# TianyiFranklinWang/MIRROR

Hardware: AMD Instinct MI355X
Metric: SSL samples/sec (slide+RNA pairs) (higher is better)
Workload: dtype bf16; 1 GPU; BASELINE c2: B=16/GPU x [4096 patch tokens x 1024-d] + [2048 genes], D=512, RNA depth 6 / 8 heads, train mode, local-batch InfoNCE; precision_policy=bf16, per_gpu_batch=16, global_batch=16, parallelism=dp1, grad_bucket_dtype=f32, step_launch=hip_graph

## Files before the change

### include/mirror_hip.h

```cpp
#ifndef MIRROR_HIP_H
#define MIRROR_HIP_H
#include <stdint.h>

#ifdef __cplusplus
extern "C" {
#endif

#define MH_OK 0
#define MH_EINVAL (-1)
#define MH_EUNSUP (-2)
#define MH_EHIP (-3)

#define MH_F32 0
#define MH_BF16 1

#define MH_ACT_NONE 0
#define MH_ACT_RELU 1
#define MH_ACT_GELU 2

typedef void* mh_stream;

const char* mh_last_error(void);
int mh_version(void);
int mh_exp_build(void);
// ... 197 lines not shown
    float* stats;
    void* qkv;
    float* attn;
    void* o;
    float* x1;
    void* u;
    void* f;
    const float* dy;
    float* dx;
    float *dw_qkv, *dw_proj, *dw_fc1, *dw_fc2, *db_qkv, *db_proj, *db_fc1, *db_fc2, *dg1, *dbe1, *dg2, *dbe2;
    void* scratch;
} mh_rna_block;
int mh_rna_block_fwd(const mh_rna_block* blk, mh_stream s);
int mh_rna_block_bwd(const mh_rna_block* blk, mh_stream s);
int64_t mh_rna_block_workspace_bytes(int B, int D, int Hh);

int mh_headattn_fwd(const void* qkv, void* out, float* attn, int B, int H, int hd, int dt, mh_stream s);
int mh_headattn_bwd(const void* qkv, const float* attn, const void* dout, void* dqkv, int B, int H, int hd,
                    int dt, mh_stream s);

int mh_add(const void* a, const void* b, void* y, int64_t n, int dt_a, int dt_b, int dt_y, mh_stream s);
int mh_cast(const void* x, void* y, int64_t n, int dt_x, int dt_y, mh_stream s);
int mh_gelu_fwd(const void* x, void* y, int64_t n, int dt_x, int dt_y, mh_stream s);
int mh_gelu_bwd(const void* x, const void* dy, void* dx, int64_t n, int dt_x, int dt_dy, int dt_dx, mh_stream s);
int mh_relu_bwd(const void* y, const void* dy, void* dx, int64_t n_per_batch, int batches, int64_t y_bs, int64_t dy_bs,
                int64_t dx_bs, int dt_y, int dt_dy, int dt_dx, mh_stream s);
int mh_noise_draws(float* out, int64_t n_uniform, int64_t n_normal, uint64_t seed, uint64_t offset, const uint64_t* dev_base, mh_stream s);
int mh_dropout(const void* x, void* y, int64_t n, float p, uint64_t seed, uint64_t offset, const uint64_t* dev_base,
               int dt_x, int dt_y, mh_stream s);
int mh_dropout_add(const float* a, const void* x, float* y, int64_t n, float p, uint64_t seed, uint64_t offset,
// ... 186 lines not shown
```

### mirror_amd/_lib.py

```python
from __future__ import annotations

import ctypes as C
import os

_HERE = os.path.dirname(os.path.abspath(__file__))
LIB_PATH = os.environ.get("MIRROR_HIP_LIB") or os.path.join(_HERE, "lib", "libmirror_hip.so")

MH_F32, MH_BF16 = 0, 1
ACT_NONE, ACT_RELU, ACT_GELU = 0, 1, 2


class GemmEpi(C.Structure):
    _fields_ = [
        ("kind", C.c_int32), ("resid", C.c_void_p),
        ("p", C.c_float), ("seed", C.c_uint64), ("offset", C.c_uint64), ("dev_base", C.c_void_p),
        ("mask", C.c_void_p), ("token", C.c_void_p), ("pos", C.c_void_p),
        ("rows_per_batch", C.c_int32), ("first", C.c_int32),
        ("tgt", C.c_void_p), ("tgt_bs", C.c_int64), ("sq", C.c_void_p),
    ]


class SkinnyWgradItem(C.Structure):
    _fields_ = [("dy", C.c_void_p), ("lddy", C.c_int64), ("x", C.c_void_p), ("ldx", C.c_int64), ("dw", C.c_void_p), ("lddw", C.c_int64),
                ("db", C.c_void_p), ("M", C.c_int32), ("N", C.c_int32), ("K", C.c_int32), ("dt_dy", C.c_int32), ("dt_x", C.c_int32)]
# ... 159 lines not shown
    "mh_kl_fwd": [P, P, P, L, F],
    "mh_kl_bwd": [P, P, P, P, P, L, F],
    "mh_symkl_fwd": [P, P, P, I, I, F],
    "mh_symkl_bwd": [P, P, P, P, P, I, I, F],
    "mh_rownorm_": [P, P, I, I, F],
    "mh_clamp_": [P, L, F, F],
    "mh_adam": [P, P, P, P, P, L, F, F, F, F, F, F, F, P, L, F, F, P, L, I, L, L],
    "mh_adam_ema": [P, P, P, P, P, L, F, F, F, F, F, F, F, P, L, F, F, P, L, I, L, L, P, P],
    "mh_ema_update_many": [P, P, I, F, P, P],
    "mh_optim_step": [P, P, P, P, P, L, P, P, P, I, F, P, L, F, F, P, L, I, L, L, P, P],
    "mh_optim_groups": [P, P, P, P, P, L, P, P, P, P, I, F, P, L, F, F, P, L, I, L, L, P, P],
    "mh_gather_many": [P, P, I],
    "mh_grad_clip": [P, L, F, F, P, P],
    "mh_rna_block_fwd": [C.POINTER(RnaBlockDesc)],
    "mh_rna_block_bwd": [C.POINTER(RnaBlockDesc)],
    "mh_loss_terms_fwd": [C.POINTER(LossTermsDesc)],
    "mh_loss_terms_bwd": [C.POINTER(LossTermsDesc)],
    "mh_surv_loss_fwd": [P, L, P, I, P, I, I, I, I, F, F, F, F, F, P, P],
    "mh_surv_loss_bwd": [P, L, P, I, P, I, I, I, I, F, F, F, F, P, I, F, P],
    "mh_surv_risk": [P, L, I, I, P],
    "mh_cindex_counts": [P, P, P, L, F, P],
    "mh_cls_ce_fwd": [P, L, P, I, I, I, F, L, P, P, I],
    "mh_cls_ce_bwd": [P, L, P, I, I, I, F, L, P, I, P],
    "mh_cls_confusion": [P, L, I, P, I, I, I, P, P],
    "mh_auroc_counts": [P, L, P, I, I, P],
    "mh_infonce_paired_fwd": [P, P, P, P, I, I, I, F, I],
    "mh_infonce_paired_bwd": [P, P, P, P, P, P, P, I, I, I, I, I],
    "mh_infonce_rows_fwd": [P, P, P, L, I, I, I, F, F, P, P, P, P],
    "mh_infonce_rows_bwd": [P, L, P, P, P, I, F, F, I, I, P, P],
    "mh_infonce_fold": [P, P, P, P, I, P, P, I, I],
# ... 107 lines not shown
```

### mirror_amd/csrc/rna_block.hip

```cpp
#include "common.h"

typedef __bf16 rb_bf16x8 __attribute__((ext_vector_type(8)));
typedef float rb_f4 __attribute__((ext_vector_type(4)));
typedef unsigned rb_u4 __attribute__((ext_vector_type(4)));
typedef unsigned rb_u2 __attribute__((ext_vector_type(2)));

namespace {

constexpr int PADK = 8;

struct Drop {
    float p;
    unsigned long long seed, offset;
};

__device__ __forceinline__ rb_f4 drop4(const Drop& d, long i) {
    if (d.p <= 0.f) return rb_f4{1.f, 1.f, 1.f, 1.f};
    const float scale = 1.f / (1.f - d.p);
    const uint32_t thr = (uint32_t)fminf(d.p * 4294967296.f, 4294967295.f);
    const uint64_t blk = (d.offset + (uint64_t)i) >> 2;
    uint32_t ctr[4] = {(uint32_t)blk, (uint32_t)(blk >> 32), 0u, 0u};
    philox4x32_10(ctr, (uint32_t)d.seed, (uint32_t)(d.seed >> 32));
    return rb_f4{ctr[0] >= thr ? scale : 0.f, ctr[1] >= thr ? scale : 0.f, ctr[2] >= thr ? scale : 0.f, ctr[3] >= thr ? scale : 0.f};
}
// ... 201 lines not shown
    Drop drop;
    int B, M;
    const bf16_t* wt;
    int Kin, epi;
    void* dx;
    const bf16_t* u;
    Drop drop2;
    int xsrc;
    const bf16_t* x_in;
    const float *xl, *stats_l, *gamma_l, *beta_l;
    float *dw, *db;
    const unsigned long long* dev_base;
    int n_dgrad, n_wgrad;
};

__device__ __forceinline__ rb_f4 gval4(const BwdArgs& g, const float* c12, int m, int n) {
    const long idx = (long)m * g.M + n;
    if (g.src == 0) return unpack4(*reinterpret_cast<const rb_u2*>(g.g_in + idx));
    rb_f4 v = *reinterpret_cast<const rb_f4*>(g.r + idx);
    if (g.src == 2) {
        const float mean = g.stats[m], rstd = g.stats[g.B + m];
        const rb_f4 xh = (*reinterpret_cast<const rb_f4*>(g.xs + idx) - mean) * rstd;
        const rb_f4 a = *reinterpret_cast<const rb_f4*>(g.dh + idx) * *reinterpret_cast<const rb_f4*>(g.gamma + n);
        v += rstd * (a - c12[m] - xh * c12[32 + m]);
    }
    return v;
}

template <int MT, int QPL>
__global__ __launch_bounds__(256) void rna_bwd_kernel(BwdArgs g) {
    extern __shared__ __attribute__((aligned(16))) char smem[];
    __shared__ float c12[64];
    const int lane = threadIdx.x & 63, wave = threadIdx.x >> 6;
    const int M = g.M;
    if (g.dev_base) {
        const unsigned long long base = *g.dev_base & ~3ull;
        g.drop.offset += base;
        g.drop2.offset += base;
    }
    const int role = (int)blockIdx.x < g.n_dgrad ? 0 : ((int)blockIdx.x < g.n_dgrad + g.n_wgrad ? 1 : 2);
// ... 15 lines not shown
                        dbt += dv[i];
                    }
            }
            g.dgamma[n] += dg;
            g.dbeta[n] += dbt;
        }
        return;
    }
    const int k0 = blockIdx.x * 16;
    const bf16_t* wp = nullptr;
    WPre pre;
    if (role == 0) {
        wp = wfrag_ptr(g.wt, M, k0, g.Kin);
        wfrag_batch(pre, wp, M / 32, wave);
    }
    if (g.src == 2) {
        for (int i0 = 0; i0 < MT * 4; i0 += 4) {
            rb_f4 xv[4][QPL], dv[4][QPL], gm[QPL];
#pragma unroll
            for (int j = 0; j < QPL; j++) {
                const int n = min(4 * (lane + 64 * j), M - 4);
                gm[j] = *reinterpret_cast<const rb_f4*>(g.gamma + n);
#pragma unroll
                for (int i = 0; i < 4; i++) {
                    const long idx = (long)min(wave + 4 * (i0 + i), g.B - 1) * M + n;
                    xv[i][j] = *reinterpret_cast<const rb_f4*>(g.xs + idx);
                    dv[i][j] = *reinterpret_cast<const rb_f4*>(g.dh + idx);
                }
            }
#pragma unroll
            for (int i = 0; i < 4; i++) {
// ... 7 lines not shown
                        s1 += a[0] + a[1] + a[2] + a[3];
                        s2 += a[0] * xh[0] + a[1] * xh[1] + a[2] * xh[2] + a[3] * xh[3];
                    }
                s1 = wave_sum(s1) / (float)M;
                s2 = wave_sum(s2) / (float)M;
                if (lane == 0 && wave + 4 * (i0 + i) < g.B) { c12[m] = s1; c12[32 + m] = s2; }
            }
        }
        __syncthreads();
    }
    if (role == 0) {
        bf16_t* sG = reinterpret_cast<bf16_t*>(smem);
        const int pitch = M + PADK;
        float* red = reinterpret_cast<float*>(smem + (size_t)MT * 16 * pitch * 2);
        const int nchunk = (M + 256 * QPL - 1) / (256 * QPL);
        for (int i0 = 0; i0 < MT * 4; i0 += 4)
            for (int c = 0; c < nchunk; c++) {
                rb_f4 v[4][QPL];
#pragma unroll
                for (int i = 0; i < 4; i++)
#pragma unroll
                    for (int j = 0; j < QPL; j++) {
                        const int m = min(wave + 4 * (i0 + i), g.B - 1), n = min(256 * QPL * c + 4 * (lane + 64 * j), M - 4);
                        v[i][j] = gval4(g, c12, m, n);
                    }
#pragma unroll
                for (int i = 0; i < 4; i++)
#pragma unroll
                    for (int j = 0; j < QPL; j++) {
                        const int m = wave + 4 * (i0 + i), n = 256 * QPL * c + 4 * (lane + 64 * j);
                        if (n >= M) continue;
                        rb_f4 o = {0.f, 0.f, 0.f, 0.f};
                        if (m < g.B) o = v[i][j] * drop4(g.drop, (long)m * M + n);
                        *reinterpret_cast<rb_u2*>(sG + m * pitch + n) = pack4(o);
                        if (g.src == 2 && g.r_out && m < g.B && (n >> 4) == (int)blockIdx.x) *reinterpret_cast<rb_f4*>(g.r_out + (long)m * M + n) = v[i][j];
                    }
            }
        __syncthreads();
        skinny_core<MT>(sG, M, wp, pre, red);
        __syncthreads();
        for (int i = threadIdx.x; i < MT * 64; i += 256) {
            const int t = i >> 6, rr = (i >> 2) & 15, c4 = 4 * (i & 3);
            const int m = 16 * t + rr, k = k0 + c4;
            if (m >= g.B || k >= g.Kin) continue;
            rb_f4 v = red_quad<MT>(red, t, rr, c4);
            const long idx = (long)m * g.Kin + k;
            if (g.epi == 1) {
                const rb_f4 uu = unpack4(*reinterpret_cast<const rb_u2*>(g.u + idx));
                v *= drop4(g.drop2, idx) * rb_f4{gelu_grad_f(uu[0]), gelu_grad_f(uu[1]), gelu_grad_f(uu[2]), gelu_grad_f(uu[3])};
            }
// ... 70 lines not shown
    }
    if (kt0 + 8 * tk >= g.Kin) return;
#pragma unroll
    for (int i = 0; i < 8; i++) {
        const int n = n0 + 8 * tn + i;
        if (n >= M) continue;
        float* dst = g.dw + (long)n * g.Kin + kt0 + 8 * tk;
        rb_f4 o0 = {acc[i][0], acc[i][1], acc[i][2], acc[i][3]}, o1 = {acc[i][4], acc[i][5], acc[i][6], acc[i][7]};
        o0 += *reinterpret_cast<const rb_f4*>(dst);
        o1 += *reinterpret_cast<const rb_f4*>(dst + 4);
        *reinterpret_cast<rb_f4*>(dst) = o0;
        *reinterpret_cast<rb_f4*>(dst + 4) = o1;
    }
}

int launch_bwd(BwdArgs a, hipStream_t s) {
    const int MT = a.B <= 16 ? 1 : 2;
    a.n_dgrad = a.dx ? mh_cdiv(a.Kin, 16) : 0;
    a.n_wgrad = a.dw ? mh_cdiv(a.M, 64) * mh_cdiv(a.Kin, 256) : 0;
    const int n_wgrad = a.n_wgrad + (a.src == 2 ? 1 : 0);
    const size_t lds_d = (size_t)MT * 16 * (a.M + PADK) * 2 + (size_t)4 * MT * 16 * 17 * 4, lds_w = 32 * 64 * 4 + 32 * 256 * 4;
    const size_t lds = lds_d > lds_w ? lds_d : lds_w;
    dim3 grid(a.n_dgrad + n_wgrad);
    if (grid.x == 0) return 0;
    static const bool attr = [] {
#define RNA_A(MT_, Q_) (void)hipFuncSetAttribute(reinterpret_cast<const void*>(&rna_bwd_kernel<MT_, Q_>), hipFuncAttributeMaxDynamicSharedMemorySize, 158 * 1024)
        RNA_A(1, 2); RNA_A(1, 4); RNA_A(1, 8); RNA_A(2, 2); RNA_A(2, 4); RNA_A(2, 8);
#undef RNA_A
        return true;
    }();
    (void)attr;
    if (lds > 158 * 1024) { mh_set_error("rna block: operand image of %zu bytes exceeds the 160 KiB of LDS", lds); return MH_EINVAL; }
#define RNA_B(MT_, Q_) hipLaunchKernelGGL((rna_bwd_kernel<MT_, Q_>), grid, dim3(256), lds, s, a)
    const int q = a.M <= 512 ? 2 : (a.M <= 1024 ? 4 : 8);
    if (MT == 1) { if (q == 2) RNA_B(1, 2); else if (q == 4) RNA_B(1, 4); else RNA_B(1, 8); }
    else { if (q == 2) RNA_B(2, 2); else if (q == 4) RNA_B(2, 4); else RNA_B(2, 8); }
#undef RNA_B
// ... 51 lines not shown
            dbt += d;
            dx[idx] = (r ? r[idx] : 0.f) + rstd * (d * gmn - c12[m] - xh * c12[32 + m]);
        }
    }
    part[0][wave][lane] = dg;
    part[1][wave][lane] = dbt;
    __syncthreads();
    if (wave == 0 && n < D) {
        dgamma[n] += part[0][0][lane] + part[0][1][lane] + part[0][2][lane] + part[0][3][lane];
        dbeta[n] += part[1][0][lane] + part[1][1][lane] + part[1][2][lane] + part[1][3][lane];
    }
}

inline long q4(long n) { return (n + 3) / 4 * 4; }

}

extern "C" int64_t mh_rna_block_workspace_bytes(int B, int D, int Hh) {
    auto al = [](long n) { return (n + 255) / 256 * 256; };
    return al(2L * B * Hh) + 3 * al(4L * B * D) + al(2L * B * D) + al(6L * B * D);
}

static int rna_check(const mh_rna_block* b, const char* who) {
    MH_REQUIRE(b, "%s: null descriptor", who);
    MH_REQUIRE(b->B >= 1 && b->B <= 32, "%s: B=%d (needs 1..32 rows)", who, b->B);
    MH_REQUIRE(b->D % 32 == 0 && b->Hh % 32 == 0 && b->D > 0 && b->Hh > 0, "%s: D=%d, Hh=%d must be multiples of 32", who, b->D, b->Hh);
    MH_REQUIRE(b->H >= 1 && b->H <= 64 && b->D % b->H == 0 && b->D <= 4096, "%s: H=%d does not divide D=%d", who, b->H, b->D);
    MH_REQUIRE(b->Hh <= 4096 && b->D <= 2048, "%s: D=%d, Hh=%d exceed the batched prologues (D <= 2048, Hh <= 4096)", who, b->D, b->Hh);
    MH_REQUIRE(b->p_drop >= 0.f && b->p_drop < 1.f && (b->offset & 3) == 0, "%s: bad dropout arguments", who);
    return MH_OK;
}

extern "C" int mh_rna_block_fwd(const mh_rna_block* b, mh_stream s) {
    if (int rc = rna_check(b, "mh_rna_block_fwd")) return rc;
    hipStream_t st = (hipStream_t)s;
    const int B = b->B, D = b->D, Hh = b->Hh;
    const unsigned long long base = b->offset;
    const Drop none{0.f, 0ull, 0ull};
    Drop d1{b->p_drop, b->seed, base}, d2{b->p_drop, b->seed, base + q4((long)B * D)}, d3{b->p_drop, b->seed, base + q4((long)B * D) + q4((long)B * Hh)};
    FwdArgs a{};
    a.B = B;
    a.dev_base = (const unsigned long long*)b->dev_base;
    a.a = b->x; a.a_f32 = 1; a.ln = 1; a.gamma = b->g1; a.beta = b->be1; a.eps = b->eps; a.stats = b->stats;
    a.w = (const bf16_t*)b->w_qkv; a.bias = b->b_qkv; a.out = b->qkv; a.out_f32 = 0; a.preact = nullptr; a.res = nullptr; a.act = MH_ACT_NONE;
    a.drop = none; a.N = 3 * D; a.K = D;
    if (int rc = launch_fwd(a, st)) return rc;
    if (int rc = mh_headattn_fwd(b->qkv, b->o, b->attn, B, b->H, D / b->H, MH_BF16, s)) return rc;
    a.a = b->o; a.a_f32 = 0; a.ln = 0; a.stats = nullptr; a.w = (const bf16_t*)b->w_proj; a.bias = b->b_proj; a.out = b->x1; a.out_f32 = 1;
    a.res = b->x; a.drop = d1; a.N = D; a.K = D;
    if (int rc = launch_fwd(a, st)) return rc;
    a.a = b->x1; a.a_f32 = 1; a.ln = 1; a.gamma = b->g2; a.beta = b->be2; a.stats = b->stats + 2 * B;
    a.w = (const bf16_t*)b->w_fc1; a.bias = b->b_fc1; a.out = b->f; a.out_f32 = 0; a.preact = (bf16_t*)b->u; a.res = nullptr; a.act = MH_ACT_GELU;
    a.drop = d2; a.N = Hh; a.K = D;
    if (int rc = launch_fwd(a, st)) return rc;
    a.a = b->f; a.a_f32 = 0; a.ln = 0; a.stats = nullptr; a.w = (const bf16_t*)b->w_fc2; a.bias = b->b_fc2; a.out = b->y; a.out_f32 = 1;
    a.preact = nullptr; a.res = b->x1; a.act = MH_ACT_NONE; a.drop = d3; a.N = D; a.K = Hh;
    if (int rc = launch_fwd(a, st)) return rc;
    MH_LAUNCH_CHECK("mh_rna_block_fwd");
    return MH_OK;
}

extern "C" int mh_rna_block_bwd(const mh_rna_block* b, mh_stream s) {
    if (int rc = rna_check(b, "mh_rna_block_bwd")) return rc;
    MH_REQUIRE(b->scratch && b->dy && b->dx, "mh_rna_block_bwd: dy, dx and scratch are required");
    hipStream_t st = (hipStream_t)s;
    const int B = b->B, D = b->D, Hh = b->Hh;
    auto al = [](long n) { return (n + 255) / 256 * 256; };
    char* ws = (char*)b->scratch;
    bf16_t* dg = (bf16_t*)ws; ws += al(2L * B * Hh);
    float* dh2 = (float*)ws; ws += al(4L * B * D);
    float* dx1 = (float*)ws; ws += al(4L * B * D);
    bf16_t* dO = (bf16_t*)ws; ws += al(2L * B * D);
    bf16_t* dqkv = (bf16_t*)ws; ws += al(6L * B * D);
    float* dh1 = (float*)ws;
    const Drop none{0.f, 0ull, 0ull};
    Drop d1{b->p_drop, b->seed, b->offset}, d2{b->p_drop, b->seed, b->offset + q4((long)B * D)},
        d3{b->p_drop, b->seed, b->offset + q4((long)B * D) + q4((long)B * Hh)};
    BwdArgs a{};
    a.dev_base = (const unsigned long long*)b->dev_base;
    a.B = B;
    a.src = 1; a.r = b->dy; a.drop = d3; a.M = D; a.wt = (const bf16_t*)b->wt_fc2; a.Kin = Hh; a.epi = 1; a.dx = dg; a.u = (const bf16_t*)b->u; a.drop2 = d2;
    a.xsrc = 0; a.x_in = (const bf16_t*)b->f; a.dw = b->dw_fc2; a.db = b->db_fc2;
    if (int rc = launch_bwd(a, st)) return rc;
    a = BwdArgs{};
    a.dev_base = (const unsigned long long*)b->dev_base;
    a.B = B; a.src = 0; a.g_in = dg; a.drop = none; a.M = Hh; a.wt = (const bf16_t*)b->wt_fc1; a.Kin = D; a.epi = 0; a.dx = dh2; a.drop2 = none;
    a.xsrc = 1; a.xl = b->x1; a.stats_l = b->stats + 2 * B; a.gamma_l = b->g2; a.beta_l = b->be2; a.dw = b->dw_fc1; a.db = b->db_fc1;
    if (int rc = launch_bwd(a, st)) return rc;
    a = BwdArgs{};
    a.dev_base = (const unsigned long long*)b->dev_base;
    a.B = B; a.src = 2; a.r = b->dy; a.dh = dh2; a.xs = b->x1; a.stats = b->stats + 2 * B; a.gamma = b->g2; a.r_out = dx1; a.dgamma = b->dg2; a.dbeta = b->dbe2;
    a.drop = d1; a.M = D; a.wt = (const bf16_t*)b->wt_proj; a.Kin = D; a.epi = 2; a.dx = dO; a.drop2 = none;
    a.xsrc = 0; a.x_in = (const bf16_t*)b->o; a.dw = b->dw_proj; a.db = b->db_proj;
    if (int rc = launch_bwd(a, st)) return rc;
    if (int rc = mh_headattn_bwd(b->qkv, b->attn, dO, dqkv, B, b->H, D / b->H, MH_BF16, s)) return rc;
    a = BwdArgs{};
    a.dev_base = (const unsigned long long*)b->dev_base;
    a.B = B; a.src = 0; a.g_in = dqkv; a.drop = none; a.M = 3 * D; a.wt = (const bf16_t*)b->wt_qkv; a.Kin = D; a.epi = 0; a.dx = dh1; a.drop2 = none;
    a.xsrc = 1; a.xl = b->x; a.stats_l = b->stats; a.gamma_l = b->g1; a.beta_l = b->be1; a.dw = b->dw_qkv; a.db = b->db_qkv;
    if (int rc = launch_bwd(a, st)) return rc;
#define RNA_L(Q_) hipLaunchKernelGGL((rna_ln_bwd_res_kernel<Q_>), dim3(mh_cdiv(D, 64)), dim3(256), 0, st, (const float*)dx1, (const float*)dh1, b->x, (const float*)b->stats, b->g1, b->dx, b->dg1, b->dbe1, B, D)
    if (D <= 512) RNA_L(2); else if (D <= 1024) RNA_L(4); else RNA_L(8);
#undef RNA_L
    MH_LAUNCH_CHECK("mh_rna_block_bwd");
    return MH_OK;
}
```

### mirror_amd/functional.py

```python
from __future__ import annotations

from dataclasses import dataclass
from typing import List, Optional, Tuple

import os

import torch
from torch.autograd import Function

from . import kernels as K
from ._lib import ACT_NONE, ACT_RELU, MH_BF16, MH_F32

f32, bf16 = torch.float32, torch.bfloat16


@dataclass(frozen=True)
class Precision:
    name: str
    mma: int
    act: torch.dtype
    pinv_mma: int
    fp8_fwd: bool = False


# ... 2080 lines not shown
        ctx.H = H
        return out

    @staticmethod
    def backward(ctx, dout):
        qkv, attn = ctx.saved_tensors
        dout = dout.contiguous()
        if dout.dtype != qkv.dtype:
            dout = K.cast(dout, qkv.dtype)
        return K.headattn_bwd(qkv, attn, dout, ctx.H), None


_RNA_FUSED = True


class RnaBlockFn(Function):

    NAMES = ("g1", "be1", "w_qkv", "b_qkv", "w_proj", "b_proj", "g2", "be2", "w_fc1", "b_fc1", "w_fc2", "b_fc2")

    @staticmethod
    def forward(ctx, x, g1, be1, wqkv, bqkv, wproj, bproj, g2, be2, w1, b1, w2, b2, H, eps, p, prec):
        masters = dict(zip(RnaBlockFn.NAMES, (g1, be1, wqkv, bqkv, wproj, bproj, g2, be2, w1, b1, w2, b2)))
        params = {}
        for k, v in masters.items():
            if v is None:
                params[k] = None
            elif k.startswith("w_"):
                params[k] = shadow(v, prec).contiguous()
            else:
                params[k] = v.detach().reshape(-1)
        B, D = x.shape
        Hh = w1.shape[0]
        st = _dropout_state
        ctx.drop = (float(p), st["seed"], st["offset"], st["base"]) if p > 0.0 else (0.0, 0, 0, None)
        if p > 0.0:
            q4 = lambda n: (n + 3) // 4 * 4
            o0 = st["offset"]
            st["offset"] += 2 * q4(B * D) + q4(B * Hh)
            _tap((B, D), p, st["seed"], o0, False)
            _tap((B, Hh), p, st["seed"], o0 + q4(B * D), False)
            _tap((B, D), p, st["seed"], o0 + q4(B * D) + q4(B * Hh), False)
        y, saved = K.rna_block_fwd(x, params, H, eps, *ctx.drop)
        ctx.masters, ctx.saved, ctx.cfg = masters, saved, (H, eps, prec)
        ctx.save_for_backward(x)
        return y

    @staticmethod
    def backward(ctx, dy):
        (x,) = ctx.saved_tensors
        H, eps, prec = ctx.cfg
        masters = ctx.masters
        params, params_t, grads, rets = {}, {}, {}, {}
        for k, v in masters.items():
            if v is None:
                params[k] = None
                continue
            if k.startswith("w_"):
                params[k] = shadow(v, prec).contiguous()
                params_t["wt_" + k[2:]] = shadow_t(v, prec)
                gk = "dw_" + k[2:]
            else:
                params[k] = v.detach().reshape(-1)
                gk = {"g1": "dg1", "be1": "dbe1", "g2": "dg2", "be2": "dbe2"}.get(k, "d" + k)
            buf, sunk = _gbuf(v, tuple(v.shape))
            grads[gk] = buf
            rets[k] = (v, buf, sunk)
        dx = K.rna_block_bwd(x, dy.contiguous().float(), params, params_t, grads, ctx.saved, H, eps, *ctx.drop)
        out = [dx]
        for k in RnaBlockFn.NAMES:
            if k in rets:
                v, buf, sunk = rets[k]
                out.append(_gret(v, buf, sunk))
            else:
                out.append(None)
        return tuple(out) + (None, None, None, None)


def rna_block(x, blk, prec: Precision, training: bool):
    a, m = blk.attn, blk.mlp
    p = float(a.proj_drop) if training else 0.0
    if not (_RNA_FUSED and prec.act == bf16 and x.dtype == f32 and K.rna_block_ok(x, x.shape[-1], m.fc1.weight.shape[0], a.num_heads)
            and float(m.drop) == float(a.proj_drop) and blk.norm1.eps == blk.norm2.eps):
        return None
    return RnaBlockFn.apply(x.contiguous(), blk.norm1.weight, blk.norm1.bias, a.qkv.weight, a.qkv.bias, a.proj.weight, a.proj.bias,
                            blk.norm2.weight, blk.norm2.bias, m.fc1.weight, m.fc1.bias, m.fc2.weight, m.fc2.bias,
                            a.num_heads, float(blk.norm1.eps), p, prec)


class ExpFn(Function):

    @staticmethod
    def forward(ctx, x):
        y = K.exp_fwd(x.detach().contiguous())
        ctx.save_for_backward(y)
        ctx.x = x
        return y

    @staticmethod
    def backward(ctx, dy):
        (y,) = ctx.saved_tensors
        dx, sunk = _gbuf_n(ctx.x, tuple(y.shape))
# ... 407 lines not shown
```

### mirror_amd/kernels.py

```python
from __future__ import annotations

import ctypes as C
import os
from typing import Optional


import torch

from . import _lib
from ._lib import ACT_GELU, ACT_NONE, ACT_RELU, MH_BF16, MH_F32, GemmDesc, MirrorHipError

_DT = {torch.float32: MH_F32, torch.bfloat16: MH_BF16}


def dt(t: torch.Tensor) -> int:
    try:
        return _DT[t.dtype]
    except KeyError:
        raise MirrorHipError(f"unsupported dtype {t.dtype} (f32 / bf16 only)") from None


_raw_stream = getattr(torch._C, "_cuda_getCurrentRawStream", None)


# ... 1273 lines not shown

def rna_block_bwd(x, dy, params: dict, params_t: dict, grads: dict, saved: dict, H: int, eps: float, p: float, seed: int, offset: int,
                  dev_base) -> torch.Tensor:
    import ctypes
    B, D = x.shape
    Hh = params["w_fc1"].shape[0]
    if dy.dtype != torch.float32 or not dy.is_contiguous() or dy.shape != x.shape:
        raise MirrorHipError("rna_block_bwd: dy must be a contiguous f32 [B, D] tensor")
    dx = torch.empty_like(x)
    scratch = torch.empty((rna_block_workspace_bytes(B, D, Hh),), device=x.device, dtype=torch.uint8)
    d = _rna_desc(B, D, Hh, H, eps, p, seed, offset, dev_base, x=x, dy=dy, dx=dx, scratch=scratch, **params, **params_t, **grads, **saved)
    _lib.call("mh_rna_block_bwd", ctypes.byref(d), stream=_stream())
    return dx


def add(a: torch.Tensor, b: torch.Tensor, out_dtype=None, out: Optional[torch.Tensor] = None) -> torch.Tensor:
    _chk(a, b, out)
    _contig(a, "add a"), _contig(b, "add b")
    if a.shape != b.shape:
        raise MirrorHipError(f"add: shapes differ {tuple(a.shape)} vs {tuple(b.shape)}")
    y = out if out is not None else torch.empty_like(a, dtype=out_dtype or a.dtype)
    _lib.call("mh_add", _p(a), _p(b), _p(y), a.numel(), dt(a), dt(b), dt(y), stream=_stream())
    return y


def lm_merge(a: torch.Tensor, b: Optional[torch.Tensor], out2: torch.Tensor, zero_cols: int) -> None:
    _chk(a, b, out2)
    rows, cols = a.numel() // a.shape[-1], a.shape[-1]
    if not (a.dtype == torch.float32 and a.is_contiguous() and (b is None or (b.dtype == torch.float32 and b.is_contiguous() and b.numel() == a.numel()))
            and out2.dim() == 2 and out2.dtype == torch.bfloat16 and out2.stride(1) == 1 and tuple(out2.shape) == (rows, cols + zero_cols)):
# ... 851 lines not shown
```

### mirror_amd/models/mirror.py

```python
from __future__ import annotations

import logging
import math
import os
from typing import Dict, Optional, Tuple

import numpy as np
import torch
from torch import nn

from .. import functional as Fn
from ..functional import FP32, BF16, POLICIES, Precision
from .._lib import ACT_NONE, MirrorHipError

_logger = logging.getLogger(__name__)
f32 = torch.float32

_DEFAULT_PRECISION: Optional[str] = None

_LM_MASKED = True


def set_precision(name: Optional[str]) -> None:
    global _DEFAULT_PRECISION
# ... 92 lines not shown
        if not gene_embed or gene_embed == "none":
            self.gene_embed = None
        else:
            self.gene_embed = nn.Parameter(torch.randn(1, embed_dim) * 0.02)
            _trunc_normal_(self.gene_embed, std=0.02)
        self.pos_drop_rate = pos_drop_rate
        self.blocks = nn.Sequential(*[
            Block(embed_dim, num_heads, mlp_ratio, qkv_bias, proj_drop_rate, norm_eps) for _ in range(depth)])
        self.norm = nn.LayerNorm(embed_dim, eps=norm_eps)
        self.precision: Optional[str] = None

    def forward(self, x):
        prec = resolve_precision(self.precision)
        x = self.embedding(x, prec, extra_bias=self.gene_embed, out_dtype=f32)
        x = Fn.dropout(x, self.pos_drop_rate, self.training)
        for blk in self.blocks:
            x = blk(x, prec)
        return Fn.layer_norm(x, self.norm.weight, self.norm.bias, self.norm.eps, out_dtype=f32)


class NystromAttention(nn.Module):

    def __init__(self, dim, dim_head=64, heads=8, num_landmarks=256, pinv_iterations=6, residual=True,
                 residual_conv_kernel=33, eps=1e-8, dropout=0.0):
        super().__init__()
        assert residual, "the reference always enables the residual conv (models/mirror.py:306)"
        inner = heads * dim_head
        self.heads, self.num_landmarks, self.pinv_iterations = heads, num_landmarks, pinv_iterations
        self.eps, self.drop = eps, dropout
        self.to_qkv = nn.Linear(dim, inner * 3, bias=False)
        self.to_out = nn.Sequential(nn.Linear(inner, dim), nn.Dropout(dropout))
        ks = residual_conv_kernel
# ... 503 lines not shown
```

Baseline: 2229 samples/s.

## Fuse RNA transformer blocks into one stack call with cross-block LN-backward join

Replaces the per-block autograd function for the RNA transformer with a single stacked function that runs all blocks forward in one library call. In backward, each block's closing layernorm-backward kernel is dropped: its residual join is folded into the next-lower block's first backward kernel, which reads the upper block's dx1 and dh1 scratch. For small rows it adds a one-pass path that computes the LN reduction and the join together. This cuts per-block kernel launches and one round trip of activation gradients through memory. The cost is a separate scratch buffer per block and more complex descriptor bookkeeping, though under hip_graph launch overhead is already low.

```diff
diff --git a/include/mirror_hip.h b/include/mirror_hip.h
--- a/include/mirror_hip.h
+++ b/include/mirror_hip.h
@@ -235,6 +235,8 @@
 int mh_rna_block_fwd(const mh_rna_block* blk, mh_stream s);
 int mh_rna_block_bwd(const mh_rna_block* blk, mh_stream s);
 int64_t mh_rna_block_workspace_bytes(int B, int D, int Hh);
+int mh_rna_stack_fwd(const mh_rna_block* blks, int L, mh_stream s);
+int mh_rna_stack_bwd(const mh_rna_block* blks, int L, mh_stream s);
 
 int mh_headattn_fwd(const void* qkv, void* out, float* attn, int B, int H, int hd, int dt, mh_stream s);
 int mh_headattn_bwd(const void* qkv, const float* attn, const void* dout, void* dqkv, int B, int H, int hd,
diff --git a/mirror_amd/_lib.py b/mirror_amd/_lib.py
--- a/mirror_amd/_lib.py
+++ b/mirror_amd/_lib.py
@@ -197,6 +197,8 @@
     "mh_grad_clip": [P, L, F, F, P, P],
     "mh_rna_block_fwd": [C.POINTER(RnaBlockDesc)],
     "mh_rna_block_bwd": [C.POINTER(RnaBlockDesc)],
+    "mh_rna_stack_fwd": [C.POINTER(RnaBlockDesc), I],
+    "mh_rna_stack_bwd": [C.POINTER(RnaBlockDesc), I],
     "mh_loss_terms_fwd": [C.POINTER(LossTermsDesc)],
     "mh_loss_terms_bwd": [C.POINTER(LossTermsDesc)],
     "mh_surv_loss_fwd": [P, L, P, I, P, I, I, I, I, F, F, F, F, F, P, P],
diff --git a/mirror_amd/csrc/rna_block.hip b/mirror_amd/csrc/rna_block.hip
--- a/mirror_amd/csrc/rna_block.hip
+++ b/mirror_amd/csrc/rna_block.hip
@@ -239,16 +239,19 @@
     int n_dgrad, n_wgrad;
 };
 
+__device__ __forceinline__ rb_f4 ln_join(rb_f4 r, rb_f4 x, rb_f4 dh, rb_f4 gamma, float mean, float rstd, float c1, float c2) {
+    const rb_f4 xh = (x - mean) * rstd;
+    const rb_f4 a = dh * gamma;
+    return r + rstd * (a - c1 - xh * c2);
+}
+
 __device__ __forceinline__ rb_f4 gval4(const BwdArgs& g, const float* c12, int m, int n) {
     const long idx = (long)m * g.M + n;
     if (g.src == 0) return unpack4(*reinterpret_cast<const rb_u2*>(g.g_in + idx));
     rb_f4 v = *reinterpret_cast<const rb_f4*>(g.r + idx);
-    if (g.src == 2) {
-        const float mean = g.stats[m], rstd = g.stats[g.B + m];
-        const rb_f4 xh = (*reinterpret_cast<const rb_f4*>(g.xs + idx) - mean) * rstd;
-        const rb_f4 a = *reinterpret_cast<const rb_f4*>(g.dh + idx) * *reinterpret_cast<const rb_f4*>(g.gamma + n);
-        v += rstd * (a - c12[m] - xh * c12[32 + m]);
-    }
+    if (g.src == 2)
+        v = ln_join(v, *reinterpret_cast<const rb_f4*>(g.xs + idx), *reinterpret_cast<const rb_f4*>(g.dh + idx),
+                    *reinterpret_cast<const rb_f4*>(g.gamma + n), g.stats[m], g.stats[g.B + m], c12[m], c12[32 + m]);
     return v;
 }
 
@@ -294,7 +297,8 @@
         wp = wfrag_ptr(g.wt, M, k0, g.Kin);
         wfrag_batch(pre, wp, M / 32, wave);
     }
-    if (g.src == 2) {
+    constexpr bool ONE_PASS = QPL <= 2;
+    if (g.src == 2 && !(ONE_PASS && role == 0)) {
         for (int i0 = 0; i0 < MT * 4; i0 += 4) {
             rb_f4 xv[4][QPL], dv[4][QPL], gm[QPL];
 #pragma unroll
@@ -332,6 +336,48 @@
         const int pitch = M + PADK;
         float* red = reinterpret_cast<float*>(smem + (size_t)MT * 16 * pitch * 2);
         const int nchunk = (M + 256 * QPL - 1) / (256 * QPL);
+        if (ONE_PASS && g.src == 2) {
+            for (int i0 = 0; i0 < MT * 4; i0 += 4) {
+                rb_f4 xv[4][QPL], dv[4][QPL], rv[4][QPL], gm[QPL];
+#pragma unroll
+                for (int j = 0; j < QPL; j++) {
+                    const int n = min(4 * (lane + 64 * j), M - 4);
+                    gm[j] = *reinterpret_cast<const rb_f4*>(g.gamma + n);
+#pragma unroll
+                    for (int i = 0; i < 4; i++) {
+                        const long idx = (long)min(wave + 4 * (i0 + i), g.B - 1) * M + n;
+                        xv[i][j] = *reinterpret_cast<const rb_f4*>(g.xs + idx);
+                        dv[i][j] = *reinterpret_cast<const rb_f4*>(g.dh + idx);
+                        rv[i][j] = *reinterpret_cast<const rb_f4*>(g.r + idx);
+                    }
+                }
+#pragma unroll
+                for (int i = 0; i < 4; i++) {
+                    const int m = wave + 4 * (i0 + i), mc = min(m, g.B - 1);
+                    const float mean = g.stats[mc], rstd = g.stats[g.B + mc];
+                    float s1 = 0.f, s2 = 0.f;
+#pragma unroll
+                    for (int j = 0; j < QPL; j++)
+                        if (4 * (lane + 64 * j) < M) {
+                            const rb_f4 xh = (xv[i][j] - mean) * rstd, a = dv[i][j] * gm[j];
+                            s1 += a[0] + a[1] + a[2] + a[3];
+                            s2 += a[0] * xh[0] + a[1] * xh[1] + a[2] * xh[2] + a[3] * xh[3];
+                        }
+                    s1 = wave_sum(s1) / (float)M;
+                    s2 = wave_sum(s2) / (float)M;
+#pragma unroll
+                    for (int j = 0; j < QPL; j++) {
+                        const int n = 4 * (lane + 64 * j);
+                        if (n >= M) continue;
+                        const rb_f4 v = ln_join(rv[i][j], xv[i][j], dv[i][j], gm[j], mean, rstd, s1, s2);
+                        rb_f4 o = {0.f, 0.f, 0.f, 0.f};
+                        if (m < g.B) o = v * drop4(g.drop, (long)m * M + n);
+                        *reinterpret_cast<rb_u2*>(sG + m * pitch + n) = pack4(o);
+                        if (g.r_out && m < g.B && (n >> 4) % g.n_dgrad == (int)blockIdx.x) *reinterpret_cast<rb_f4*>(g.r_out + (long)m * M + n) = v;
+                    }
+                }
+            }
+        } else
         for (int i0 = 0; i0 < MT * 4; i0 += 4)
             for (int c = 0; c < nchunk; c++) {
                 rb_f4 v[4][QPL];
@@ -351,7 +397,7 @@
                         rb_f4 o = {0.f, 0.f, 0.f, 0.f};
                         if (m < g.B) o = v[i][j] * drop4(g.drop, (long)m * M + n);
                         *reinterpret_cast<rb_u2*>(sG + m * pitch + n) = pack4(o);
-                        if (g.src == 2 && g.r_out && m < g.B && (n >> 4) == (int)blockIdx.x) *reinterpret_cast<rb_f4*>(g.r_out + (long)m * M + n) = v[i][j];
+                        if (g.src == 2 && g.r_out && m < g.B && (n >> 4) % g.n_dgrad == (int)blockIdx.x) *reinterpret_cast<rb_f4*>(g.r_out + (long)m * M + n) = v[i][j];
                     }
             }
         __syncthreads();
@@ -452,13 +498,18 @@
     }
 }
 
+size_t bwd_lds(int B, int M) {
+    const int MT = B <= 16 ? 1 : 2;
+    const size_t lds_d = (size_t)MT * 16 * (M + PADK) * 2 + (size_t)4 * MT * 16 * 17 * 4, lds_w = 32 * 64 * 4 + 32 * 256 * 4;
+    return lds_d > lds_w ? lds_d : lds_w;
+}
+
 int launch_bwd(BwdArgs a, hipStream_t s) {
     const int MT = a.B <= 16 ? 1 : 2;
     a.n_dgrad = a.dx ? mh_cdiv(a.Kin, 16) : 0;
     a.n_wgrad = a.dw ? mh_cdiv(a.M, 64) * mh_cdiv(a.Kin, 256) : 0;
     const int n_wgrad = a.n_wgrad + (a.src == 2 ? 1 : 0);
-    const size_t lds_d = (size_t)MT * 16 * (a.M + PADK) * 2 + (size_t)4 * MT * 16 * 17 * 4, lds_w = 32 * 64 * 4 + 32 * 256 * 4;
-    const size_t lds = lds_d > lds_w ? lds_d : lds_w;
+    const size_t lds = bwd_lds(a.B, a.M);
     dim3 grid(a.n_dgrad + n_wgrad);
     if (grid.x == 0) return 0;
     static const bool attr = [] {
@@ -540,12 +591,27 @@
 
 inline long q4(long n) { return (n + 3) / 4 * 4; }
 
-}
-
-extern "C" int64_t mh_rna_block_workspace_bytes(int B, int D, int Hh) {
-    auto al = [](long n) { return (n + 255) / 256 * 256; };
-    return al(2L * B * Hh) + 3 * al(4L * B * D) + al(2L * B * D) + al(6L * B * D);
-}
+struct Ws {
+    bf16_t *dg, *dO, *dqkv;
+    float *dh2, *dx1, *dh1, *dyj;
+    long bytes;
+    Ws(void* scratch, int B, int D, int Hh) {
+        auto al = [](long n) { return (n + 255) / 256 * 256; };
+        char* p = (char*)scratch;
+        dg = (bf16_t*)p; p += al(2L * B * Hh);
+        dh2 = (float*)p; p += al(4L * B * D);
+        dx1 = (float*)p; p += al(4L * B * D);
+        dO = (bf16_t*)p; p += al(2L * B * D);
+        dqkv = (bf16_t*)p; p += al(6L * B * D);
+        dh1 = (float*)p; p += al(4L * B * D);
+        dyj = (float*)p; p += al(4L * B * D);
+        bytes = p - (char*)scratch;
+    }
+};
+
+}
+
+extern "C" int64_t mh_rna_block_workspace_bytes(int B, int D, int Hh) { return Ws(nullptr, B, D, Hh).bytes; }
 
 static int rna_check(const mh_rna_block* b, const char* who) {
     MH_REQUIRE(b, "%s: null descriptor", who);
@@ -557,8 +623,8 @@
     return MH_OK;
 }
 
-extern "C" int mh_rna_block_fwd(const mh_rna_block* b, mh_stream s) {
-    if (int rc = rna_check(b, "mh_rna_block_fwd")) return rc;
+static int rna_fwd_one(const mh_rna_block* b, mh_stream s, const char* who) {
+    if (int rc = rna_check(b, who)) return rc;
     hipStream_t st = (hipStream_t)s;
     const int B = b->B, D = b->D, Hh = b->Hh;
     const unsigned long long base = b->offset;
@@ -581,31 +647,47 @@
     if (int rc = launch_fwd(a, st)) return rc;
     a.a = b->f; a.a_f32 = 0; a.ln = 0; a.stats = nullptr; a.w = (const bf16_t*)b->w_fc2; a.bias = b->b_fc2; a.out = b->y; a.out_f32 = 1;
     a.preact = nullptr; a.res = b->x1; a.act = MH_ACT_NONE; a.drop = d3; a.N = D; a.K = Hh;
-    if (int rc = launch_fwd(a, st)) return rc;
+    return launch_fwd(a, st);
+}
+
+extern "C" int mh_rna_block_fwd(const mh_rna_block* b, mh_stream s) {
+    if (int rc = rna_fwd_one(b, s, "mh_rna_block_fwd")) return rc;
     MH_LAUNCH_CHECK("mh_rna_block_fwd");
     return MH_OK;
 }
 
-extern "C" int mh_rna_block_bwd(const mh_rna_block* b, mh_stream s) {
-    if (int rc = rna_check(b, "mh_rna_block_bwd")) return rc;
-    MH_REQUIRE(b->scratch && b->dy && b->dx, "mh_rna_block_bwd: dy, dx and scratch are required");
+extern "C" int mh_rna_stack_fwd(const mh_rna_block* blks, int L, mh_stream s) {
+    MH_REQUIRE(blks && L >= 1, "mh_rna_stack_fwd: needs at least one block");
+    for (int l = 0; l < L; l++) {
+        MH_REQUIRE(l == 0 || blks[l].x == blks[l - 1].y, "mh_rna_stack_fwd: block %d does not read block %d's output", l, l - 1);
+        if (int rc = rna_fwd_one(blks + l, s, "mh_rna_stack_fwd")) return rc;
+    }
+    MH_LAUNCH_CHECK("mh_rna_stack_fwd");
+    return MH_OK;
+}
+
+static int rna_bwd_one(const mh_rna_block* b, const mh_rna_block* above, bool close, mh_stream s, const char* who) {
+    if (int rc = rna_check(b, who)) return rc;
+    MH_REQUIRE(b->scratch && (above || b->dy) && (!close || b->dx), "%s: dy, dx and scratch are required", who);
+    MH_REQUIRE(!above || (above->B == b->B && above->D == b->D && above->scratch), "%s: stacked blocks differ in B or D", who);
     hipStream_t st = (hipStream_t)s;
     const int B = b->B, D = b->D, Hh = b->Hh;
-    auto al = [](long n) { return (n + 255) / 256 * 256; };
-    char* ws = (char*)b->scratch;
-    bf16_t* dg = (bf16_t*)ws; ws += al(2L * B * Hh);
-    float* dh2 = (float*)ws; ws += al(4L * B * D);
-    float* dx1 = (float*)ws; ws += al(4L * B * D);
-    bf16_t* dO = (bf16_t*)ws; ws += al(2L * B * D);
-    bf16_t* dqkv = (bf16_t*)ws; ws += al(6L * B * D);
-    float* dh1 = (float*)ws;
+    const Ws w(b->scratch, B, D, Hh);
+    bf16_t *dg = w.dg, *dO = w.dO, *dqkv = w.dqkv;
+    float *dh2 = w.dh2, *dx1 = w.dx1, *dh1 = w.dh1;
+    const float* dy = above ? w.dyj : b->dy;
     const Drop none{0.f, 0ull, 0ull};
     Drop d1{b->p_drop, b->seed, b->offset}, d2{b->p_drop, b->seed, b->offset + q4((long)B * D)},
         d3{b->p_drop, b->seed, b->offset + q4((long)B * D) + q4((long)B * Hh)};
     BwdArgs a{};
     a.dev_base = (const unsigned long long*)b->dev_base;
     a.B = B;
-    a.src = 1; a.r = b->dy; a.drop = d3; a.M = D; a.wt = (const bf16_t*)b->wt_fc2; a.Kin = Hh; a.epi = 1; a.dx = dg; a.u = (const bf16_t*)b->u; a.drop2 = d2;
+    if (above) {
+        const Ws wa(above->scratch, B, D, above->Hh);
+        a.src = 2; a.r = wa.dx1; a.dh = wa.dh1; a.xs = above->x; a.stats = above->stats; a.gamma = above->g1; a.r_out = w.dyj;
+        a.dgamma = above->dg1; a.dbeta = above->dbe1;
+    } else { a.src = 1; a.r = b->dy; }
+    a.drop = d3; a.M = D; a.wt = (const bf16_t*)b->wt_fc2; a.Kin = Hh; a.epi = 1; a.dx = dg; a.u = (const bf16_t*)b->u; a.drop2 = d2;
     a.xsrc = 0; a.x_in = (const bf16_t*)b->f; a.dw = b->dw_fc2; a.db = b->db_fc2;
     if (int rc = launch_bwd(a, st)) return rc;
     a = BwdArgs{};
@@ -615,7 +697,7 @@
     if (int rc = launch_bwd(a, st)) return rc;
     a = BwdArgs{};
     a.dev_base = (const unsigned long long*)b->dev_base;
-    a.B = B; a.src = 2; a.r = b->dy; a.dh = dh2; a.xs = b->x1; a.stats = b->stats + 2 * B; a.gamma = b->g2; a.r_out = dx1; a.dgamma = b->dg2; a.dbeta = b->dbe2;
+    a.B = B; a.src = 2; a.r = dy; a.dh = dh2; a.xs = b->x1; a.stats = b->stats + 2 * B; a.gamma = b->g2; a.r_out = dx1; a.dgamma = b->dg2; a.dbeta = b->dbe2;
     a.drop = d1; a.M = D; a.wt = (const bf16_t*)b->wt_proj; a.Kin = D; a.epi = 2; a.dx = dO; a.drop2 = none;
     a.xsrc = 0; a.x_in = (const bf16_t*)b->o; a.dw = b->dw_proj; a.db = b->db_proj;
     if (int rc = launch_bwd(a, st)) return rc;
@@ -625,9 +707,25 @@
     a.B = B; a.src = 0; a.g_in = dqkv; a.drop = none; a.M = 3 * D; a.wt = (const bf16_t*)b->wt_qkv; a.Kin = D; a.epi = 0; a.dx = dh1; a.drop2 = none;
     a.xsrc = 1; a.xl = b->x; a.stats_l = b->stats; a.gamma_l = b->g1; a.beta_l = b->be1; a.dw = b->dw_qkv; a.db = b->db_qkv;
     if (int rc = launch_bwd(a, st)) return rc;
+    if (!close) return MH_OK;
 #define RNA_L(Q_) hipLaunchKernelGGL((rna_ln_bwd_res_kernel<Q_>), dim3(mh_cdiv(D, 64)), dim3(256), 0, st, (const float*)dx1, (const float*)dh1, b->x, (const float*)b->stats, b->g1, b->dx, b->dg1, b->dbe1, B, D)
     if (D <= 512) RNA_L(2); else if (D <= 1024) RNA_L(4); else RNA_L(8);
 #undef RNA_L
+    return MH_OK;
+}
+
+extern "C" int mh_rna_block_bwd(const mh_rna_block* b, mh_stream s) {
+    if (int rc = rna_bwd_one(b, nullptr, true, s, "mh_rna_block_bwd")) return rc;
     MH_LAUNCH_CHECK("mh_rna_block_bwd");
     return MH_OK;
 }
+
+extern "C" int mh_rna_stack_bwd(const mh_rna_block* blks, int L, mh_stream s) {
+    MH_REQUIRE(blks && L >= 1, "mh_rna_stack_bwd: needs at least one block");
+    for (int l = L - 1; l >= 0; l--) {
+        MH_REQUIRE(l == L - 1 || blks[l].scratch != blks[l + 1].scratch, "mh_rna_stack_bwd: blocks %d and %d share their scratch", l, l + 1);
+        if (int rc = rna_bwd_one(blks + l, l == L - 1 ? nullptr : blks + l + 1, l == 0, s, "mh_rna_stack_bwd")) return rc;
+    }
+    MH_LAUNCH_CHECK("mh_rna_stack_bwd");
+    return MH_OK;
+}
diff --git a/mirror_amd/functional.py b/mirror_amd/functional.py
--- a/mirror_amd/functional.py
+++ b/mirror_amd/functional.py
@@ -2118,77 +2118,83 @@
 _RNA_FUSED = True
 
 
-class RnaBlockFn(Function):
+class RnaStackFn(Function):
 
     NAMES = ("g1", "be1", "w_qkv", "b_qkv", "w_proj", "b_proj", "g2", "be2", "w_fc1", "b_fc1", "w_fc2", "b_fc2")
 
     @staticmethod
-    def forward(ctx, x, g1, be1, wqkv, bqkv, wproj, bproj, g2, be2, w1, b1, w2, b2, H, eps, p, prec):
-        masters = dict(zip(RnaBlockFn.NAMES, (g1, be1, wqkv, bqkv, wproj, bproj, g2, be2, w1, b1, w2, b2)))
-        params = {}
-        for k, v in masters.items():
-            if v is None:
-                params[k] = None
-            elif k.startswith("w_"):
-                params[k] = shadow(v, prec).contiguous()
-            else:
-                params[k] = v.detach().reshape(-1)
+    def forward(ctx, x, H, eps, ps, prec, *tensors):
+        n = len(RnaStackFn.NAMES)
+        masters = [dict(zip(RnaStackFn.NAMES, tensors[i:i + n])) for i in range(0, len(tensors), n)]
         B, D = x.shape
-        Hh = w1.shape[0]
         st = _dropout_state
-        ctx.drop = (float(p), st["seed"], st["offset"], st["base"]) if p > 0.0 else (0.0, 0, 0, None)
-        if p > 0.0:
-            q4 = lambda n: (n + 3) // 4 * 4
-            o0 = st["offset"]
-            st["offset"] += 2 * q4(B * D) + q4(B * Hh)
-            _tap((B, D), p, st["seed"], o0, False)
-            _tap((B, Hh), p, st["seed"], o0 + q4(B * D), False)
-            _tap((B, D), p, st["seed"], o0 + q4(B * D) + q4(B * Hh), False)
-        y, saved = K.rna_block_fwd(x, params, H, eps, *ctx.drop)
-        ctx.masters, ctx.saved, ctx.cfg = masters, saved, (H, eps, prec)
-        ctx.save_for_backward(x)
+        q4 = lambda n: (n + 3) // 4 * 4
+        params, drops = [], []
+        for m, p in zip(masters, ps):
+            params.append({k: None if v is None else (shadow(v, prec).contiguous() if k.startswith("w_") else v.detach().reshape(-1))
+                           for k, v in m.items()})
+            Hh = m["w_fc1"].shape[0]
+            drops.append((float(p), st["seed"], st["offset"], st["base"]) if p > 0.0 else (0.0, 0, 0, None))
+            if p > 0.0:
+                o0 = st["offset"]
+                st["offset"] += 2 * q4(B * D) + q4(B * Hh)
+                _tap((B, D), p, st["seed"], o0, False)
+                _tap((B, Hh), p, st["seed"], o0 + q4(B * D), False)
+                _tap((B, D), p, st["seed"], o0 + q4(B * D) + q4(B * Hh), False)
+        y, saved = K.rna_stack_fwd(x, params, H, eps, drops)
+        ctx.masters, ctx.saved, ctx.cfg, ctx.drops = masters, saved, (H, eps, prec), drops
         return y
 
     @staticmethod
     def backward(ctx, dy):
-        (x,) = ctx.saved_tensors
         H, eps, prec = ctx.cfg
-        masters = ctx.masters
-        params, params_t, grads, rets = {}, {}, {}, {}
-        for k, v in masters.items():
-            if v is None:
-                params[k] = None
-                continue
-            if k.startswith("w_"):
-                params[k] = shadow(v, prec).contiguous()
-                params_t["wt_" + k[2:]] = shadow_t(v, prec)
-                gk = "dw_" + k[2:]
-            else:
-                params[k] = v.detach().reshape(-1)
-                gk = {"g1": "dg1", "be1": "dbe1", "g2": "dg2", "be2": "dbe2"}.get(k, "d" + k)
-            buf, sunk = _gbuf(v, tuple(v.shape))
-            grads[gk] = buf
-            rets[k] = (v, buf, sunk)
-        dx = K.rna_block_bwd(x, dy.contiguous().float(), params, params_t, grads, ctx.saved, H, eps, *ctx.drop)
-        out = [dx]
-        for k in RnaBlockFn.NAMES:
-            if k in rets:
-                v, buf, sunk = rets[k]
-                out.append(_gret(v, buf, sunk))
-            else:
-                out.append(None)
-        return tuple(out) + (None, None, None, None)
+        params, params_t, grads, rets = [], [], [], []
+        for m in ctx.masters:
+            pr, pt, gr = {}, {}, {}
+            for k, v in m.items():
+                if v is None:
+                    pr[k] = None
+                    rets.append(None)
+                    continue
+                if k.startswith("w_"):
+                    pr[k] = shadow(v, prec).contiguous()
+                    pt["wt_" + k[2:]] = shadow_t(v, prec)
+                    gk = "dw_" + k[2:]
+                else:
+                    pr[k] = v.detach().reshape(-1)
+                    gk = {"g1": "dg1", "be1": "dbe1", "g2": "dg2", "be2": "dbe2"}.get(k, "d" + k)
+                buf, sunk = _gbuf(v, tuple(v.shape))
+                gr[gk] = buf
+                rets.append((v, buf, sunk))
+            params.append(pr), params_t.append(pt), grads.append(gr)
+        dx = K.rna_stack_bwd(dy.contiguous().float(), params, params_t, grads, ctx.saved, H, eps, ctx.drops)
+        return (dx, None, None, None, None) + tuple(None if r is None else _gret(*r) for r in rets)
+
+
+def _rna_fused_ok(x, blk, prec: Precision) -> bool:
+    a, m = blk.attn, blk.mlp
+    return bool(_RNA_FUSED and prec.act == bf16 and x.dtype == f32 and K.rna_block_ok(x, x.shape[-1], m.fc1.weight.shape[0], a.num_heads)
+                and float(m.drop) == float(a.proj_drop) and blk.norm1.eps == blk.norm2.eps)
+
+
+def rna_stack(x, blocks, prec: Precision, training: bool):
+    blocks = list(blocks)
+    if not blocks or not all(_rna_fused_ok(x, b, prec) for b in blocks):
+        return None
+    b0 = blocks[0]
+    if any(b.attn.num_heads != b0.attn.num_heads or b.norm1.eps != b0.norm1.eps for b in blocks):
+        return None
+    tensors = []
+    for b in blocks:
+        a, m = b.attn, b.mlp
+        tensors += [b.norm1.weight, b.norm1.bias, a.qkv.weight, a.qkv.bias, a.proj.weight, a.proj.bias,
+                    b.norm2.weight, b.norm2.bias, m.fc1.weight, m.fc1.bias, m.fc2.weight, m.fc2.bias]
+    ps = tuple(float(b.attn.proj_drop) if training else 0.0 for b in blocks)
+    return RnaStackFn.apply(x.contiguous(), b0.attn.num_heads, float(b0.norm1.eps), ps, prec, *tensors)
 
 
 def rna_block(x, blk, prec: Precision, training: bool):
-    a, m = blk.attn, blk.mlp
-    p = float(a.proj_drop) if training else 0.0
-    if not (_RNA_FUSED and prec.act == bf16 and x.dtype == f32 and K.rna_block_ok(x, x.shape[-1], m.fc1.weight.shape[0], a.num_heads)
-            and float(m.drop) == float(a.proj_drop) and blk.norm1.eps == blk.norm2.eps):
-        return None
-    return RnaBlockFn.apply(x.contiguous(), blk.norm1.weight, blk.norm1.bias, a.qkv.weight, a.qkv.bias, a.proj.weight, a.proj.bias,
-                            blk.norm2.weight, blk.norm2.bias, m.fc1.weight, m.fc1.bias, m.fc2.weight, m.fc2.bias,
-                            a.num_heads, float(blk.norm1.eps), p, prec)
+    return rna_stack(x, [blk], prec, training)
 
 
 class ExpFn(Function):
diff --git a/mirror_amd/kernels.py b/mirror_amd/kernels.py
--- a/mirror_amd/kernels.py
+++ b/mirror_amd/kernels.py
@@ -1311,6 +1311,56 @@
     return dx
 
 
+def _rna_saved(B, D, Hh, H, dev) -> dict:
+    bf, f = torch.bfloat16, torch.float32
+    return {"stats": torch.empty((4, B), device=dev, dtype=f), "qkv": torch.empty((B, 3 * D), device=dev, dtype=bf),
+            "attn": torch.empty((B, H, H), device=dev, dtype=f), "o": torch.empty((B, D), device=dev, dtype=bf),
+            "x1": torch.empty((B, D), device=dev, dtype=f), "u": torch.empty((B, Hh), device=dev, dtype=bf),
+            "f": torch.empty((B, Hh), device=dev, dtype=bf)}
+
+
+def rna_stack_fwd(x, params: list, H: int, eps: float, drops: list):
+    import ctypes
+    B, D = x.shape
+    descs = (_lib.RnaBlockDesc * len(params))()
+    saved, keep = [], []
+    for l, (pr, drop) in enumerate(zip(params, drops)):
+        for k in ("w_qkv", "w_proj", "w_fc1", "w_fc2"):
+            if pr[k].dtype != torch.bfloat16 or not pr[k].is_contiguous():
+                raise MirrorHipError(f"rna_stack_fwd: block {l}: {k} must be a contiguous bf16 matrix")
+        Hh = pr["w_fc1"].shape[0]
+        sv = _rna_saved(B, D, Hh, H, x.device)
+        y = torch.empty((B, D), device=x.device, dtype=torch.float32)
+        descs[l] = _rna_desc(B, D, Hh, H, eps, *drop, x=x, y=y, **pr, **sv)
+        sv["x"] = x
+        saved.append(sv)
+        keep.append(y)
+        x = y
+    _lib.call("mh_rna_stack_fwd", descs, len(params), stream=_stream())
+    return x, saved
+
+
+def rna_stack_bwd(dy, params: list, params_t: list, grads: list, saved: list, H: int, eps: float, drops: list) -> torch.Tensor:
+    B, D = saved[0]["x"].shape
+    if dy.dtype != torch.float32 or not dy.is_contiguous() or tuple(dy.shape) != (B, D):
+        raise MirrorHipError("rna_stack_bwd: dy must be a contiguous f32 [B, D] tensor")
+    L = len(params)
+    descs = (_lib.RnaBlockDesc * L)()
+    dx = torch.empty_like(dy)
+    scratch = []
+    for l in range(L):
+        Hh = params[l]["w_fc1"].shape[0]
+        scratch.append(torch.empty((rna_block_workspace_bytes(B, D, Hh),), device=dy.device, dtype=torch.uint8))
+        ends = {}
+        if l == L - 1:
+            ends["dy"] = dy
+        if l == 0:
+            ends["dx"] = dx
+        descs[l] = _rna_desc(B, D, Hh, H, eps, *drops[l], scratch=scratch[l], **ends, **params[l], **params_t[l], **grads[l], **saved[l])
+    _lib.call("mh_rna_stack_bwd", descs, L, stream=_stream())
+    return dx
+
+
 def add(a: torch.Tensor, b: torch.Tensor, out_dtype=None, out: Optional[torch.Tensor] = None) -> torch.Tensor:
     _chk(a, b, out)
     _contig(a, "add a"), _contig(b, "add b")
diff --git a/mirror_amd/models/mirror.py b/mirror_amd/models/mirror.py
--- a/mirror_amd/models/mirror.py
+++ b/mirror_amd/models/mirror.py
@@ -130,8 +130,12 @@
         prec = resolve_precision(self.precision)
         x = self.embedding(x, prec, extra_bias=self.gene_embed, out_dtype=f32)
         x = Fn.dropout(x, self.pos_drop_rate, self.training)
-        for blk in self.blocks:
-            x = blk(x, prec)
+        y = Fn.rna_stack(x, self.blocks, prec, self.training)
+        if y is None:
+            for blk in self.blocks:
+                x = blk(x, prec)
+        else:
+            x = y
         return Fn.layer_norm(x, self.norm.weight, self.norm.bias, self.norm.eps, out_dtype=f32)
 
 
```

Result: no change. 2220 samples/s (-0.4%).
